# mirage/decompress

Hardware: AMD Instinct MI355X
Metric: MiB/s inflate over N zlib streams (uncompressed bytes / wall second) (higher is better)
Workload: dtype u8; 1 GPU; C2: 4096 x 256 KiB zlib streams per GPU, dynamic Huffman (libz level 6; even streams = slices of the reference's test/corpus, odd = order-2 Markov ASCII text, 64 symbols, seed 0xC2 + i, SURVEY 8(d)), Zl.Inf.Ns semantics, one stream per pair of wavefronts (decoder + copier); streams_per_gpu=4096, stream_bytes=262144, unique_streams=4096

## Files before the change

decompress_amd/csrc/inflate_util.hpp:

```cpp
#pragma once
#include <hip/hip_runtime.h>
#include <type_traits>
#include <stdint.h>

#include "mdeflate.h"

namespace md {
namespace wv {

constexpr int kWave = 64;
__device__ __forceinline__ uint32_t uni(uint32_t v) { return __builtin_amdgcn_readfirstlane(v); }

#define MD_LDS __attribute__((address_space(3)))
typedef MD_LDS uint32_t lds_u32;
typedef MD_LDS uint16_t lds_u16;
typedef MD_LDS uint8_t lds_u8;
typedef uint64_t u64_u __attribute__((aligned(1), may_alias));
typedef uint32_t u32_u __attribute__((aligned(1), may_alias));
typedef uint16_t u16_u __attribute__((aligned(1), may_alias));

enum { P_ENSURE = 0, P_DECODE1, P_DECODE2, P_EMIT_A, P_FAR, P_NEAR, P_ADLER, P_HEADER, P_NEAR_FAST, P_NEAR_SLOW, P_NEAR_UPD, P_NEAR_LOAD, P_HDR_LENS, P_HDR_LIT, P_FAR_REC, P_FAR_LOAD, P_WAIT_DEC, P_WAIT_COPY, P_COUNT };
enum { C_ROUNDS = 0, C_PASSES, C_LANES, C_TOKENS, C_SLOTS, C_NEAR_IT,
       C_END_CHAIN, C_END_FIT, C_END_RECORDS, C_END_STAGE, C_END_EOB, C_LONG_NEAR, C_FAR_SPILL, C_COUNT };
template <bool ON>
struct Prof {
  static constexpr bool on = true;
  uint64_t t0;
  uint64_t acc[P_COUNT];
  uint32_t cnt[C_COUNT];
  __device__ __forceinline__ void init() {
    for (int i = 0; i < P_COUNT; i++) acc[i] = 0;
    for (int i = 0; i < C_COUNT; i++) cnt[i] = 0;
    t0 = clock64();
  }
  __device__ __forceinline__ void tick(int i) {
    uint64_t t = clock64();
    acc[i] += t - t0;
    t0 = t;
  }
  __device__ __forceinline__ void tick_lds(int i) {
    __builtin_amdgcn_s_waitcnt(0xc07f);
    tick(i);
  }
  __device__ __forceinline__ void tick_all(int i) {
    __builtin_amdgcn_s_waitcnt(0);
    tick(i);
  }
  __device__ __forceinline__ void count(int i, uint32_t n = 1) { cnt[i] += n; }
};
template <>
struct Prof<false> {
  static constexpr bool on = false;
  __device__ __forceinline__ void init() {}
  __device__ __forceinline__ void tick(int) {}
  __device__ __forceinline__ void tick_lds(int) {}
  __device__ __forceinline__ void tick_all(int) {}
  __device__ __forceinline__ void count(int, uint32_t = 1) {}
};

__device__ __forceinline__ uint32_t wave_incl_scan(uint32_t x) {
  uint32_t v = x;
  v += (uint32_t)__builtin_amdgcn_update_dpp(0, (int)v, 0x111, 0xf, 0xf, false);
  v += (uint32_t)__builtin_amdgcn_update_dpp(0, (int)v, 0x112, 0xf, 0xf, false);
  v += (uint32_t)__builtin_amdgcn_update_dpp(0, (int)v, 0x114, 0xf, 0xf, false);
  v += (uint32_t)__builtin_amdgcn_update_dpp(0, (int)v, 0x118, 0xf, 0xf, false);
  v += (uint32_t)__builtin_amdgcn_update_dpp(0, (int)v, 0x142, 0xa, 0xf, false);
  v += (uint32_t)__builtin_amdgcn_update_dpp(0, (int)v, 0x143, 0xc, 0xf, false);
  return v;
}
__device__ __forceinline__ uint32_t wave_sum(uint32_t v) {
  return (uint32_t)__builtin_amdgcn_readlane((int)wave_incl_scan(v), 63);
}
__device__ __forceinline__ uint32_t wave_excl_scan(uint32_t v, uint32_t) { return wave_incl_scan(v) - v; }
__device__ __forceinline__ uint32_t wave_shr1(uint32_t v) { return (uint32_t)__builtin_amdgcn_update_dpp(0, (int)v, 0x138, 0xf, 0xf, false); }
__device__ __forceinline__ uint32_t rdlane(uint32_t v, uint32_t l) {
  return __builtin_amdgcn_readlane(v, __builtin_amdgcn_readfirstlane(l));
}

__device__ __forceinline__ uint64_t out_ld64(const uint8_t *p) {
  return __builtin_nontemporal_load(reinterpret_cast<const u64_u *>(p));
}
__device__ __forceinline__ uint32_t out_ld8(const uint8_t *p) { return __builtin_nontemporal_load(p); }
__device__ __forceinline__ uint64_t out_ld_guard(const uint8_t *g, uint32_t x, uint32_t n, uint32_t cap) {
  if (x + 8 <= cap) return out_ld64(g + x);
  uint64_t v = 0;
  for (uint32_t j = 0; j < n && j < 8; j++) v |= (uint64_t)out_ld8(g + x + j) << (8 * j);
  return v;
}
__device__ __forceinline__ uint64_t lds_ld64(const lds_u8 *p) { return *reinterpret_cast<const MD_LDS u64_u *>(p); }

__device__ __forceinline__ void lds_put(lds_u8 *p, uint64_t v, uint32_t n) {
  const uint32_t lo = (uint32_t)v, hi = (uint32_t)(v >> 32);
  if (n >= 4) {
    const uint32_t k = n - 4;
    const uint32_t t = k >= 4 ? hi : __builtin_amdgcn_alignbyte(hi, lo, k);
    *reinterpret_cast<MD_LDS u32_u *>(p) = lo;
    *reinterpret_cast<MD_LDS u32_u *>(p + k) = t;
  } else {
    *p = (uint8_t)lo;
    if (n > 1) *reinterpret_cast<MD_LDS u16_u *>(p + n - 2) = (uint16_t)(lo >> (8 * (n - 2)));
  }
}

}
}
```

decompress_amd/csrc/inflate_wave_core.hpp:

```cpp
#pragma once
#include <stdlib.h>
#include "inflate_util.hpp"
#include "internal.hpp"

#if !defined(MD_RMAX) || !defined(MD_STAGE)
#error "define MD_RMAX and MD_STAGE before inflate_wave_core.hpp"
#endif

namespace md {
namespace wv {

constexpr uint32_t S = 264;
constexpr uint32_t SMIN = 48;
constexpr uint32_t KMAX = 64;
#ifndef MD_EMIT_SPLIT
#define MD_EMIT_SPLIT 1
#endif
#if defined(MD_DEBUG_KNOWN_BOUNDS)
#undef MD_EMIT_SPLIT
#define MD_EMIT_SPLIT 0
#endif
#ifndef MD_SPLIT_B
#define MD_SPLIT_B 4
#endif
#ifndef MD_RUNIN_NUM
#define MD_RUNIN_NUM 3
#define MD_RUNIN_DEN 2
#endif
constexpr uint32_t RUNIN_NUM = MD_RUNIN_NUM, RUNIN_DEN = MD_RUNIN_DEN;
constexpr uint32_t PASSES = 5;
constexpr uint32_t PASS_BITS = 1600, PASSES_MAX = 16;
constexpr uint32_t RMAX = MD_RMAX;
constexpr uint32_t STAGE = MD_STAGE;
constexpr uint32_t WIN_WORDS = 544;

constexpr uint32_t kLitSize = 852, kDistSize = 592;
constexpr uint32_t kLitRootMax = 512;
constexpr uint32_t kLitSubB = 0;
constexpr uint32_t kDistB = kLitSize - kLitRootMax;
constexpr uint32_t kLitB = kDistB + kDistSize;
constexpr uint32_t kStopEobI = kLitB + kLitRootMax;
constexpr uint32_t kStopBadI = kStopEobI + 2;
constexpr uint32_t kLutWords = kStopBadI + 2;
constexpr uint32_t kTbMask = 0xffe00000u;
constexpr uint32_t kLoopy = 0x100u;
static_assert(kDistB % 2 == 0 && kLitB % 2 == 0 && kStopEobI % 2 == 0 && kLutWords == 1448, "even table bases");
constexpr uint32_t kStEob = 100, kStTrunc = 101;
constexpr uint32_t kCountMatch = 1u << 20;
constexpr uint32_t kNearBit = 0x8000u;

struct Mail {
  uint32_t emitted;
  uint32_t copied;
  uint32_t kind;
  uint32_t total;
  uint32_t x;
  uint32_t stuck;
  uint32_t a, b;
};
constexpr uint32_t kJobRound = 0, kJobStored = 1, kJobQuit = 2, kJobEmit = 3;
constexpr uint32_t kHxUni = 4 * 64;
struct Smem {
  uint32_t win[WIN_WORDS];
  uint32_t lut[kLutWords];
  uint32_t mrec[RMAX];
  uint16_t mpos[RMAX];
  alignas(16) uint8_t stage[STAGE + 16];
  uint16_t list[RMAX];
  Mail mail;
};
struct HScratch {
  uint8_t lens[384];
  uint16_t work[320];
  uint32_t ctr;
};
#if MD_RMAX == 576 && MD_STAGE == 5248
static_assert(sizeof(Smem) <= 17920, "9 streams (18 wavefronts) per CU: 160 KiB / 9, in whole 512-byte units");
#endif
static_assert(RMAX % 64 == 0 && STAGE % 16 == 0 && RMAX * 2 >= (kHxUni + 6) * 4, "record rows, staging chunks, the emit job's words in `list`");
constexpr uint32_t kHScratchAt = 1136;
static_assert(kHScratchAt >= 4 + 572 + 8 && kHScratchAt % 16 == 0 && kHScratchAt + sizeof(HScratch) <= WIN_WORDS * 4, "header scratch lives behind the header's bits");
typedef MD_LDS Smem lds_smem;
typedef MD_LDS HScratch lds_hscratch;
__device__ __forceinline__ lds_hscratch *hscratch_of(lds_smem *sm) {
  return reinterpret_cast<lds_hscratch *>(reinterpret_cast<lds_u8 *>(sm->win) + kHScratchAt);
}

__device__ __forceinline__ uint32_t mk_entry(uint32_t n, uint32_t xb, uint32_t val8, uint32_t nbits, uint32_t tb) {
  return n | (xb << 5) | (val8 << 9) | (nbits << 17) | (tb << 21);
}
__device__ __forceinline__ uint32_t e_n(uint32_t e) { return e & 31; }
__device__ __forceinline__ uint32_t e_xb(uint32_t e) { return (e >> 5) & 15; }
__device__ __forceinline__ uint32_t e_val(uint32_t e) { return (e >> 9) & 255; }
__device__ __forceinline__ uint32_t e_tb(uint32_t e) { return e >> 21; }
__device__ __forceinline__ bool e_link(uint32_t e) { return e_tb(e) < kLitB && e_tb(e) != kDistB; }
__device__ __forceinline__ uint32_t e_root(uint32_t lroot) { return mk_entry(0, 0, 0, lroot, kLitB); }
__device__ __forceinline__ uint32_t lit_leaf(uint32_t sym, uint32_t codelen, uint32_t lroot, uint32_t droot) {
  if (sym < 256) return mk_entry(codelen, 0, sym, lroot, kLitB);
  if (sym == 256) return mk_entry(codelen, 0, 0, 0, kStopEobI);
  const uint32_t l = (sym - 257) & 31;
  const uint32_t xb = (l >= 8 && l < 28) ? (l - 4) >> 2 : 0;
  const uint32_t base3 = l < 8 ? l : l < 28 ? (4 + (l & 3)) << xb : l == 28 ? 255 : 0;
  return mk_entry(codelen + xb, xb, base3, droot, kDistB);
}
__device__ __forceinline__ uint32_t dist_leaf(uint32_t dv, uint32_t codelen, uint32_t lroot) {
  dv &= 31;
  if (dv >= 30) return mk_entry(codelen, 0, 0, 0, kStopBadI);
  const uint32_t xb = dv >= 4 ? (dv - 2) >> 1 : 0;
  const uint32_t m = dv < 4 ? dv : ((dv & 1) | 2);
  return mk_entry(codelen + xb, xb, m, lroot, kLitB);
}
__device__ __forceinline__ uint32_t dist_value(uint32_t m, uint32_t xb, uint32_t x) { return (m << xb) + 1 + x; }

struct Window {
  uint32_t w[8], wx;
  uint32_t base;
#ifdef MD_DEBUG_KNOWN_BOUNDS
  uint32_t kb_round, kb_sid;
#endif
  __device__ __forceinline__ void fetch(const uint8_t *__restrict__ body, uint32_t nbytes, uint32_t b, uint32_t lane) {
    base = b;
    const uint32_t off = b + lane * 32;
#pragma unroll
    for (int k = 0; k < 8; k++) w[k] = 0;
    if (off + 32 <= nbytes) __builtin_memcpy(w, body + off, 32);
    else if (off < nbytes)
      for (uint32_t k = 0; k < 32 && off + k < nbytes; k++) w[k >> 2] |= (uint32_t)body[off + k] << (8 * (k & 3));
    wx = 0;
    if (lane < WIN_WORDS - 512) {
      const uint32_t ox = b + 2048 + lane * 4;
      if (ox + 4 <= nbytes) __builtin_memcpy(&wx, body + ox, 4);
      else if (ox < nbytes)
        for (uint32_t k = 0; k < 4 && ox + k < nbytes; k++) wx |= (uint32_t)body[ox + k] << (8 * k);
    }
  }
  __device__ __forceinline__ void put(lds_u32 *win, uint32_t lane) const {
    lds_u32 *dst = win + lane * 8;
#pragma unroll
    for (int k = 0; k < 8; k++) dst[k] = w[k];
    if (lane < WIN_WORDS - 512) win[512 + lane] = wx;
  }
  __device__ __forceinline__ void ensure(lds_u32 *win, const uint8_t *__restrict__ body, uint32_t nbytes, uint32_t b, uint32_t lane) {
    if (base != b) fetch(body, nbytes, b, lane);
    put(win, lane);
    base = 0xffffffffu;
  }
};
__device__ __forceinline__ uint32_t peek(const lds_u32 *win, uint32_t p) {
  const lds_u32 *q = reinterpret_cast<const lds_u32 *>(reinterpret_cast<const lds_u8 *>(win) + ((p >> 3) & ~3u));
  return __builtin_amdgcn_alignbit(q[1], q[0], p & 31);
}
__device__ __forceinline__ uint32_t lut_at(const lds_u32 *lut, uint32_t tb, uint32_t idx) {
  return *reinterpret_cast<const lds_u32 *>(reinterpret_cast<const lds_u8 *>(lut) + ((tb + idx) << 2));
}

struct UBits {
  const lds_u32 *win;
  uint64_t buf;
  uint32_t n;
  uint32_t wp;
  __device__ __forceinline__ void init(const lds_u32 *w, uint32_t bp) {
    win = w;
    wp = bp >> 5;
    buf = ((uint64_t)uni(win[wp]) | ((uint64_t)uni(win[wp + 1]) << 32)) >> (bp & 31);
    n = 64 - (bp & 31);
    wp += 2;
  }
  __device__ __forceinline__ uint32_t pos() const { return wp * 32 - n; }
  __device__ __forceinline__ void fill() {
    if (n <= 32) {
      buf |= (uint64_t)uni(win[wp]) << n;
      n += 32;
      wp++;
    }
  }
  __device__ __forceinline__ uint32_t peekb(uint32_t k) const { return (uint32_t)buf & ((1u << k) - 1); }
  __device__ __forceinline__ void drop(uint32_t k) {
    buf >>= k;
    n -= k;
  }
};

struct Canon {
  uint32_t cnt[16];
  uint32_t first[16];
  uint32_t offs[16];
  uint32_t max, min, root, left;
};
__device__ __forceinline__ uint32_t lane_rank(uint64_t m) {
  return __builtin_amdgcn_mbcnt_hi((uint32_t)(m >> 32), __builtin_amdgcn_mbcnt_lo((uint32_t)m, 0));
}
template <int K>
__device__ __forceinline__ void canon_counts(const uint32_t (&len)[K], uint32_t rootpref, Canon &c) {
#pragma unroll
  for (int l = 1; l < 16; l++) {
    uint32_t n = 0;
#pragma unroll
    for (int k = 0; k < K; k++) n += (uint32_t)__builtin_popcountll(__ballot(len[k] == (uint32_t)l));
    c.cnt[l] = n;
  }
  c.cnt[0] = 0;
  c.max = 0;
  c.min = 16;
#pragma unroll
  for (int l = 15; l >= 1; l--) {
    if (c.cnt[l] && c.max == 0) c.max = l;
    if (c.cnt[l]) c.min = l;
  }
  int left = 1;
  bool over = false;
  uint32_t code = 0, off = 0;
  c.first[0] = 0;
  c.offs[0] = 0;
#pragma unroll
  for (int l = 1; l < 16; l++) {
    left = (left << 1) - (int)c.cnt[l];
    over = over || left < 0;
    code = (code + c.cnt[l - 1]) << 1;
    c.first[l] = code;
    c.offs[l] = off;
    off += c.cnt[l];
  }
  c.left = over ? 0xffffffffu : (uint32_t)left;
  uint32_t root = rootpref;
  if (root > c.max) root = c.max;
  if (root < c.min) root = c.min;
  c.root = root;
}

template <int K, class LEAF>
__device__ __forceinline__ bool build_walk(const uint32_t (&len)[K], const Canon &c, lds_u32 *lut, uint32_t tb0, uint32_t sub0,
                                           uint32_t size, lds_hscratch *hs, uint32_t lane, uint32_t zero_entry, LEAF leaf) {
  const uint32_t root = c.root, rmask = (1u << root) - 1;
  uint32_t rev[K];
#pragma unroll
  for (int k = 0; k < K; k++) rev[k] = 0;
#pragma unroll
  for (int l = 1; l < 16; l++) {
    if (c.cnt[l]) {
      uint32_t base = 0;
#pragma unroll
      for (int k = 0; k < K; k++) {
        const uint64_t m = __ballot(len[k] == (uint32_t)l);
        if (len[k] == (uint32_t)l) {
          const uint32_t rank = base + lane_rank(m);
          rev[k] = __brev(c.first[l] + rank) >> (32 - l);
          hs->work[c.offs[l] + rank] = (uint16_t)(lane + 64 * k);
        }
        base += (uint32_t)__builtin_popcountll(m);
      }
    }
  }
  const uint32_t nroot = 1u << root;
  for (uint32_t i = lane; i < nroot; i += kWave) lut[tb0 + i] = 0;
  if (lane == 0) hs->ctr = 0;
  if (c.max > root) {
#pragma unroll
    for (int k = 0; k < K; k++)
      if (len[k] > root)
        __hip_atomic_fetch_max(&lut[tb0 + (rev[k] & rmask)], len[k], __ATOMIC_RELAXED, __HIP_MEMORY_SCOPE_WORKGROUP);
  }
  for (uint32_t i = lane; i < nroot; i += kWave) {
    const uint32_t v = lut[tb0 + i];
    uint32_t e;
    if (v) {
      const uint32_t sub = v - root;
      const uint32_t off = __hip_atomic_fetch_add(&hs->ctr, 1u << sub, __ATOMIC_RELAXED, __HIP_MEMORY_SCOPE_WORKGROUP);
      e = mk_entry(root, 0, 0, sub, (sub0 + off) & 2047);
    } else {
      const uint32_t cw = __brev(i) >> (32 - root);
      uint32_t fl = 0, ft = 0;
#pragma unroll
      for (int l = 15; l >= 1; l--) {
        if (c.cnt[l] && (uint32_t)l <= root) {
          const uint32_t t = (cw >> (root - l)) - c.first[l];
          if (t < c.cnt[l]) {
            fl = l;
            ft = c.offs[l] + t;
          }
        }
      }
      e = fl ? leaf((uint32_t)hs->work[ft], fl) : zero_entry;
    }
    lut[tb0 + i] = e;
  }
  const uint32_t used = nroot + uni(hs->ctr);
  if (used > size) return false;
  if (c.max > root) {
#pragma unroll
    for (int k = 0; k < K; k++) {
      if (len[k] > root) {
        const uint32_t link = lut[tb0 + (rev[k] & rmask)];
        const uint32_t sub = (link >> 17) & 15, tb = link >> 21;
        const uint32_t e = leaf(lane + 64 * k, len[k] - root);
        for (uint32_t j = rev[k] >> root; j < (1u << sub); j += 1u << (len[k] - root)) lut[tb + j] = e;
      }
    }
  }
  return true;
}

constexpr uint64_t kZig0 = 16ull | 17ull << 5 | 18ull << 10 | 0ull << 15 | 8ull << 20 | 7ull << 25 | 9ull << 30 | 6ull << 35 |
                           10ull << 40 | 5ull << 45 | 11ull << 50 | 4ull << 55;
constexpr uint64_t kZig1 = 12ull | 3ull << 5 | 13ull << 10 | 2ull << 15 | 14ull << 20 | 1ull << 25 | 15ull << 30;

template <class PF>
__device__ __noinline__ int dynamic_tables(lds_smem *sm, uint32_t bp_arg, uint32_t tot_arg, uint32_t lane, uint32_t *bp_out,
                                           uint32_t *lroot_out, PF &pf) {
  const uint32_t bp = uni(bp_arg), tot = uni(tot_arg);
  const lds_u32 *win = (const lds_u32 *)sm->win;
  lds_hscratch *hs = hscratch_of(sm);
  UBits ub;
  ub.init(win, bp);
  if ((int32_t)(tot - ub.pos()) < 14) return MD_UNEXPECTED_END_OF_INPUT;
  const uint32_t hlit = ub.peekb(5) + 257;
  ub.drop(5);
  const uint32_t hdist = ub.peekb(5) + 1;
  ub.drop(5);
  const uint32_t hclen = ub.peekb(4) + 4;
  ub.drop(4);
  uint32_t cl[1] = {0};
  for (uint32_t i = 0; i < hclen; i++) {
    ub.fill();
    if ((int32_t)(tot - ub.pos()) < 3) return MD_UNEXPECTED_END_OF_INPUT;
    const uint32_t v = ub.peekb(3);
    ub.drop(3);
    const uint32_t z = (uint32_t)((i < 12 ? kZig0 >> (5 * i) : kZig1 >> (5 * (i - 12))) & 31);
    if (lane == z) cl[0] = v;
  }
  Canon cc;
  canon_counts<1>(cl, 7, cc);
  uint32_t cmaxl, t_lo, t_hi;
  if (cc.max == 0) {
    cmaxl = 1;
    t_lo = lane == 0 ? (1u << 8) : 0xffffu;
    t_hi = 0xffffu;
  } else {
    if (cc.left != 0) return MD_INVALID_DICTIONARY;
    cmaxl = cc.max;
#pragma unroll
    for (int l = 1; l < 8; l++) {
      const uint64_t m = __ballot(cl[0] == (uint32_t)l);
      if (cl[0] == (uint32_t)l) hs->work[cc.offs[l] + lane_rank(m)] = (uint16_t)lane;
    }
    uint32_t t[2];
#pragma unroll
    for (int h = 0; h < 2; h++) {
      const uint32_t i = lane + 64 * h;
      const uint32_t cw = __brev(i & ((1u << cmaxl) - 1)) >> (32 - cmaxl);
      uint32_t fl = 0, ft = 0;
#pragma unroll
      for (int l = 7; l >= 1; l--) {
        if (cc.cnt[l] && (uint32_t)l <= cmaxl) {
          const uint32_t x = (cw >> (cmaxl - l)) - cc.first[l];
          if (x < cc.cnt[l]) {
            fl = l;
            ft = cc.offs[l] + x;
          }
        }
      }
      t[h] = fl ? ((uint32_t)hs->work[ft] | (fl << 8)) : 0xffffu;
    }
    t_lo = t[0];
    t_hi = t[1];
  }
  const uint32_t max_res = hlit + hdist;
  for (uint32_t x = lane; x < 384; x += kWave) hs->lens[x] = 0;
  auto run_lengths = [&](auto checked) -> int {
    constexpr bool CHECK = decltype(checked)::value;
    uint32_t i = 0, prev = 0;
    while (i < max_res) {
      ub.fill();
      if (CHECK && (int32_t)(tot - ub.pos()) < (int32_t)cmaxl) return MD_UNEXPECTED_END_OF_INPUT;
      const uint32_t idx = ub.peekb(cmaxl);
      const uint32_t e_lo = __builtin_amdgcn_readlane(t_lo, idx & 63), e_hi = __builtin_amdgcn_readlane(t_hi, idx & 63);
      const uint32_t e = idx < 64 ? e_lo : e_hi;
      if (e == 0xffffu) return MD_INVALID_DICTIONARY;
      const uint32_t sym = e & 0xff;
      ub.drop(e >> 8);
      if (sym < 16) {
        hs->lens[i] = (uint8_t)sym;
        prev = sym;
        i++;
      } else {
        const uint32_t nb = sym == 16 ? 2 : sym == 17 ? 3 : 7;
        if (sym == 16 && i == 0) return MD_INVALID_DICTIONARY;
        ub.fill();
        if (CHECK && (int32_t)(tot - ub.pos()) < (int32_t)nb) return MD_UNEXPECTED_END_OF_INPUT;
        const uint32_t copy = ub.peekb(nb) + (sym == 18 ? 11 : 3);
        ub.drop(nb);
        const uint32_t val = sym == 16 ? prev : 0;
        if (i + copy > max_res) return MD_INVALID_DICTIONARY;
        if (val)
          for (uint32_t x = lane; x < copy; x += kWave) hs->lens[i + x] = (uint8_t)val;
        prev = val;
        i += copy;
      }
    }
    return MD_OK;
  };
  {
    const bool plenty = (int32_t)(tot - ub.pos()) >= 316 * 14 + 64;
    const int rc = plenty ? run_lengths(std::false_type{}) : run_lengths(std::true_type{});
    if (rc != MD_OK) return rc;
  }
  *bp_out = ub.pos();
  pf.tick_lds(P_HDR_LENS);
  if (uni(hs->lens[256]) == 0) return MD_INVALID_DICTIONARY;
  uint32_t ll[5], dl[1];
#pragma unroll
  for (int k = 0; k < 5; k++) ll[k] = lane + 64 * k < hlit ? (uint32_t)hs->lens[lane + 64 * k] : 0u;
  dl[0] = lane < hdist ? (uint32_t)hs->lens[hlit + lane] : 0u;
  Canon cl_, cd_;
  canon_counts<5>(ll, 9, cl_);
  canon_counts<1>(dl, 6, cd_);
  if (cl_.left == 0xffffffffu || (cl_.left > 0 && cl_.max != 1)) return MD_INVALID_DICTIONARY;
  const uint32_t lroot = cl_.root;
  uint32_t droot;
  lds_u32 *lut = (lds_u32 *)sm->lut;
  if (cd_.max == 0) {
    droot = 1;
  } else {
    if (cd_.left == 0xffffffffu || (cd_.left > 0 && cd_.max != 1)) return MD_INVALID_DICTIONARY;
    droot = cd_.root;
  }
  if (!build_walk<5>(ll, cl_, lut, kLitB, kLitSubB, kLitSize, hs, lane, e_root(lroot),
                     [=](uint32_t sym, uint32_t codelen) { return lit_leaf(sym, codelen, lroot, droot); }))
    return MD_INVALID_DICTIONARY;
  pf.tick_lds(P_HDR_LIT);
  if (cd_.max == 0) {
    if (lane == 0) {
      lut[kDistB] = dist_leaf(0, 1, lroot);
      lut[kDistB + 1] = mk_entry(0, 0, 0, 0, kStopBadI);
    }
  } else if (!build_walk<1>(dl, cd_, lut, kDistB, kDistB + (1u << droot), kDistSize, hs, lane, e_root(lroot),
                            [=](uint32_t sym, uint32_t codelen) { return dist_leaf(sym, codelen, lroot); }))
    return MD_INVALID_DICTIONARY;
  const bool loopy = cl_.left > 0 || (cd_.max != 0 && cd_.left > 0);
  *lroot_out = lroot | (loopy ? kLoopy : 0u);
  return MD_OK;
}

__device__ __noinline__ void fixed_tables(lds_smem *sm, uint32_t lane, uint32_t *lroot_out) {
  lds_hscratch *hs = hscratch_of(sm);
  uint32_t ll[5], dl[1];
#pragma unroll
  for (int k = 0; k < 5; k++) {
    const uint32_t n = lane + 64 * k;
    ll[k] = n < 144 ? 8 : n < 256 ? 9 : n < 280 ? 7 : n < 288 ? 8 : 0;
  }
  dl[0] = lane < 32 ? 5 : 0;
  Canon cl_, cd_;
  canon_counts<5>(ll, 9, cl_);
  canon_counts<1>(dl, 6, cd_);
  const uint32_t lroot = cl_.root, droot = cd_.root;
  lds_u32 *lut = (lds_u32 *)sm->lut;
  build_walk<5>(ll, cl_, lut, kLitB, kLitSubB, kLitSize, hs, lane, e_root(lroot),
                [=](uint32_t sym, uint32_t codelen) { return lit_leaf(sym, codelen, lroot, droot); });
  build_walk<1>(dl, cd_, lut, kDistB, kDistB + (1u << droot), kDistSize, hs, lane, e_root(lroot),
                [=](uint32_t sym, uint32_t codelen) { return dist_leaf(sym, codelen, lroot); });
  *lroot_out = lroot;
}

struct Cursor {
  uint32_t w0, w1, w2, wa;
  __device__ __forceinline__ void init(const lds_u32 *win, uint32_t p) {
    wa = (p >> 5) << 2;
    const lds_u32 *q = reinterpret_cast<const lds_u32 *>(reinterpret_cast<const lds_u8 *>(win) + wa);
    w0 = q[0];
    w1 = q[1];
    w2 = q[2];
  }
  __device__ __forceinline__ uint32_t peek(uint32_t p) const { return __builtin_amdgcn_alignbit(w1, w0, p); }
  __device__ __forceinline__ void seek(const lds_u32 *win, uint32_t pn) {
    const uint32_t wan = (pn >> 5) << 2;
    const bool ge = wan != wa;
    w0 = ge ? w1 : w0;
    w1 = ge ? w2 : w1;
    wa = wan;
    w2 = *reinterpret_cast<const lds_u32 *>(reinterpret_cast<const lds_u8 *>(win) + wa + 8);
  }
};
__device__ __forceinline__ uint32_t lut_step(const lds_u32 *lut, uint32_t e, uint32_t w) {
  return lut_at(lut, e >> 21, __builtin_amdgcn_ubfe(w, 0, e >> 17));
}

template <bool COUNT, bool BUDGET, bool MID = false>
__device__ __forceinline__ void sync_pass(const lds_u32 *win, const lds_u32 *lut, uint32_t lroot, bool go, uint32_t start,
                                          uint32_t limit, uint32_t &end, uint32_t &stop, uint32_t &nb, uint32_t mthr = 0,
                                          uint32_t *midp = nullptr, uint32_t *midcnt = nullptr) {
  if (go) {
    uint32_t p = start, e = e_root(lroot), cnt = 0;
    uint32_t mp = 0xffffffffu, mc = 0;
    bool got = false;
    if (MID && start >= mthr) {
      mp = start;
      got = true;
    }
    if (p < limit) {
      const uint32_t thr = (kLitB << 21) | limit;
      uint32_t slot = 0, key;
      Cursor c;
      c.init(win, start);
      do {
        const uint32_t w = c.peek(p);
        const uint32_t en = lut_step(lut, e, w);
        const uint32_t n = e_n(en);
        if (COUNT) {
          const uint32_t xb = e_xb(en);
          const uint32_t len1 = e_val(en) + __builtin_amdgcn_ubfe(w, n - xb, xb) + (kCountMatch + 2);
          cnt += (e_tb(en) == kLitB ? 1u : 0u) + (e_tb(en) == kDistB ? len1 : 0u);
        }
        p += n;
        if (MID) {
          const bool cross = (e_tb(en) == kLitB) & !got & (p >= mthr);
          mp = cross ? p : mp;
          mc = cross ? cnt : mc;
          got = got | cross;
        }
        c.seek(win, p);
        e = en;
        key = (en & kTbMask) | p;
        if (BUDGET && ++slot >= KMAX && e_tb(en) == kLitB) break;
      } while (key < thr);
    }
    end = p;
    stop = e_tb(e) >= kStopEobI ? e_tb(e) : 0u;
    if (COUNT) nb = cnt;
    if (MID) {
      *midp = mp;
      *midcnt = mc;
    }
  }
}

struct LaneOut {
  uint32_t endp;
  uint32_t stopc;
  uint32_t bytes;
  uint32_t nm;
};

__device__ __noinline__ uint32_t slow_token(const lds_u32 *win, const lds_u32 *lut, uint32_t lroot, uint32_t ptok, uint32_t q,
                                            uint32_t tot, uint32_t cap) {
  uint32_t p = ptok;
  uint32_t w = peek(win, p);
  uint32_t e = lut_step(lut, e_root(lroot), w);
  if (e_link(e)) {
    p += e_n(e);
    w = peek(win, p);
    e = lut_step(lut, e, w);
  }
  uint32_t n = e_n(e), xb = e_xb(e), ntb = e_tb(e);
  uint32_t pn = p + n;
  if (pn > tot) return MD_UNEXPECTED_END_OF_INPUT;
  if (ntb == kStopEobI) return kStEob | (pn << 8);
  if (ntb != kDistB) {
    if (q >= cap) return MD_UNEXPECTED_END_OF_OUTPUT;
    return kStTrunc;
  }
  const uint32_t mlen = e_val(e) + 3 + __builtin_amdgcn_ubfe(w, n - xb, xb);
  p = pn;
  w = peek(win, p);
  e = lut_step(lut, e, w);
  if (e_tb(e) == kStopBadI && e_n(e) == 0) return MD_INVALID_DISTANCE_CODE;
  if (e_link(e)) {
    p += e_n(e);
    w = peek(win, p);
    e = lut_step(lut, e, w);
  }
  n = e_n(e), xb = e_xb(e);
  pn = p + n;
  if (pn > tot) return MD_UNEXPECTED_END_OF_INPUT;
  if (e_tb(e) == kStopBadI) return MD_INVALID_DISTANCE_CODE;
  const uint32_t d = dist_value(e_val(e), xb, __builtin_amdgcn_ubfe(w, n - xb, xb));
  const uint32_t lim = q < 32768u ? q : 32768u;
  if (d > lim) return MD_INVALID_DISTANCE;
  if (mlen > cap - q) return MD_UNEXPECTED_END_OF_OUTPUT;
  return kStTrunc;
}

template <bool CHECKED, bool BUDGET>
__device__ __forceinline__ void emit_pass(const lds_u32 *win, const lds_u32 *lut, uint32_t lroot, lds_u32 *mrec,
                                          lds_u16 *mpos, lds_u8 *stage, uint32_t rec0, uint32_t tot, bool go, uint32_t start,
                                          uint32_t limit, uint32_t q0, uint32_t rb, uint32_t R0, uint32_t cap, LaneOut &lo) {
  uint32_t p = start, ptok = start, e = e_root(lroot);
  uint32_t q = q0, rec = rec0, mlen = 0;
  bool stopped = false;
  const uint32_t qlim = rb + STAGE - 16;
  const uint32_t qmax = cap < qlim ? cap : qlim;
  if (go && p < limit) {
    const uint32_t thr = (kLitB << 21) | limit;
    uint32_t slot = 0, key;
    Cursor c;
    c.init(win, start);
    do {
      const uint32_t w = c.peek(p);
      const uint32_t en = lut_step(lut, e, w);
      const uint32_t n = e_n(en), xb = e_xb(en), ntb = e_tb(en);
      const uint32_t x = __builtin_amdgcn_ubfe(w, n - xb, xb);
      const uint32_t pn = p + n;
      const bool to_root = ntb == kLitB, is_len = ntb == kDistB;
      const bool mat = to_root & (mlen != 0), lit = to_root & (mlen == 0);
      const uint32_t d1 = (e_val(en) << xb) + x;
      if (CHECKED) {
        const uint32_t lim = q < 32768u ? q : 32768u;
        const uint32_t need = mat ? mlen : 1u;
        stopped = (ntb >= kStopEobI) | (pn > tot) | (mat & (d1 >= lim)) | (to_root & (q + need > qmax));
        if (stopped) break;
      }
      stage[lit ? q - rb : STAGE + 15] = (uint8_t)(en >> 9);
      if (mat) {
        mrec[rec] = ((mlen - 3) << 16) | ((q - d1 + mlen > R0 + 1) ? kNearBit : 0u) | d1;
        mpos[rec] = (uint16_t)(q - rb);
        rec++;
      }
      q += to_root ? (mlen > 1u ? mlen : 1u) : 0u;
      mlen = is_len ? e_val(en) + 3 + x : to_root ? 0u : mlen;
      p = pn;
      ptok = to_root ? pn : ptok;
      c.seek(win, p);
      e = en;
      key = (en & kTbMask) | p;
      if (BUDGET && ++slot >= KMAX && to_root) break;
    } while (key < thr);
    if (!CHECKED) stopped = e_tb(e) >= kStopEobI;
  }
  uint32_t stopc = 0, endp = p;
  if (go && stopped) {
    const uint32_t r = slow_token(win, lut, lroot, ptok, q, tot, cap);
    stopc = r & 0xffu;
    endp = stopc == kStEob ? r >> 8 : ptok;
  }
  if (go) {
    lo.endp = endp;
    lo.stopc = stopc;
    lo.bytes = q - q0;
    lo.nm = rec - rec0;
  }
}

}
}
```

Baseline: 249,200 MiB/s.

## Decode dynamic Huffman header from registers instead of LDS

The dynamic-header bit reader now loads up to 128 window words into two VGPRs per lane and reads them back with readlane, replacing scalar LDS loads on every fill. Code-length-code fields are decoded in parallel, with each lane picking its own 3-bit field through an inverse zigzag table. Run-length decoded code lengths are written into registers with writelane and lane masks rather than into an LDS byte array, and the distance lengths are realigned with ds_bpermute. This removes LDS round-trips and waits from the serial header decode, at the cost of more register pressure and some readlane/writelane overhead.

```diff
diff --git a/decompress_amd/csrc/inflate_util.hpp b/decompress_amd/csrc/inflate_util.hpp
--- a/decompress_amd/csrc/inflate_util.hpp
+++ b/decompress_amd/csrc/inflate_util.hpp
@@ -77,6 +77,9 @@
   return __builtin_amdgcn_readlane(v, __builtin_amdgcn_readfirstlane(l));
 }
 
+extern "C" __device__ uint32_t md_llvm_writelane(uint32_t v, uint32_t l, uint32_t old) __asm("llvm.amdgcn.writelane.i32");
+__device__ __forceinline__ uint32_t wrlane(uint32_t old, uint32_t v, uint32_t l) { return md_llvm_writelane(v, l, old); }
+
 __device__ __forceinline__ uint64_t out_ld64(const uint8_t *p) {
   return __builtin_nontemporal_load(reinterpret_cast<const u64_u *>(p));
 }
diff --git a/decompress_amd/csrc/inflate_wave_core.hpp b/decompress_amd/csrc/inflate_wave_core.hpp
--- a/decompress_amd/csrc/inflate_wave_core.hpp
+++ b/decompress_amd/csrc/inflate_wave_core.hpp
@@ -70,7 +70,6 @@
   Mail mail;
 };
 struct HScratch {
-  uint8_t lens[384];
   uint16_t work[320];
   uint32_t ctr;
 };
@@ -78,8 +77,16 @@
 static_assert(sizeof(Smem) <= 17920, "9 streams (18 wavefronts) per CU: 160 KiB / 9, in whole 512-byte units");
 #endif
 static_assert(RMAX % 64 == 0 && STAGE % 16 == 0 && RMAX * 2 >= (kHxUni + 6) * 4, "record rows, staging chunks, the emit job's words in `list`");
+constexpr uint32_t kHdrBitsMax = 14 + 19 * 3 + 316 * 7;
+constexpr uint32_t kHdrReuseBits = 4096;
+constexpr uint32_t kHdrWordMax = (kHdrReuseBits + 3) / 32;
+constexpr uint32_t kHdrWords = 128;
+static_assert(31 + kHdrBitsMax + 14 + 64 <= kHdrWords * 32, "start phase, header, a last peek and the bit buffer's read-ahead");
 constexpr uint32_t kHScratchAt = 1136;
-static_assert(kHScratchAt >= 4 + 572 + 8 && kHScratchAt % 16 == 0 && kHScratchAt + sizeof(HScratch) <= WIN_WORDS * 4, "header scratch lives behind the header's bits");
+static_assert(kHScratchAt >= (kHdrWordMax + 1) * 4 + (kHdrBitsMax + 7) / 8 + 8 && kHScratchAt % 16 == 0 &&
+                  kHScratchAt + sizeof(HScratch) <= WIN_WORDS * 4,
+              "header scratch lives behind the header's bits");
+static_assert(kHdrWordMax + kHdrWords <= WIN_WORDS, "the header's register copy stays inside the window");
 typedef MD_LDS Smem lds_smem;
 typedef MD_LDS HScratch lds_hscratch;
 __device__ __forceinline__ lds_hscratch *hscratch_of(lds_smem *sm) {
@@ -155,21 +162,35 @@
 }
 
 struct UBits {
-  const lds_u32 *win;
+  uint32_t hw[2];
+  uint32_t w0;
   uint64_t buf;
   uint32_t n;
   uint32_t wp;
-  __device__ __forceinline__ void init(const lds_u32 *w, uint32_t bp) {
-    win = w;
-    wp = bp >> 5;
-    buf = ((uint64_t)uni(win[wp]) | ((uint64_t)uni(win[wp + 1]) << 32)) >> (bp & 31);
-    n = 64 - (bp & 31);
+  __device__ __forceinline__ uint32_t word(uint32_t i) const {
+    const uint32_t a = __builtin_amdgcn_readlane(hw[0], i & 63), b = __builtin_amdgcn_readlane(hw[1], i & 63);
+    return i < 64 ? a : b;
+  }
+  __device__ __forceinline__ void load(const lds_u32 *win, uint32_t bp, uint32_t lane) {
+    w0 = bp >> 5;
+#pragma unroll
+    for (int j = 0; j < 2; j++) {
+      const uint32_t w = w0 + lane + 64 * j;
+      hw[j] = win[w < WIN_WORDS ? w : WIN_WORDS - 1];
+    }
+    seek(bp & 31);
+  }
+  __device__ __forceinline__ void seek(uint32_t p) {
+    wp = p >> 5;
+    buf = ((uint64_t)word(wp) | ((uint64_t)word(wp + 1) << 32)) >> (p & 31);
+    n = 64 - (p & 31);
     wp += 2;
   }
-  __device__ __forceinline__ uint32_t pos() const { return wp * 32 - n; }
+  __device__ __forceinline__ uint32_t hpos() const { return wp * 32 - n; }
+  __device__ __forceinline__ uint32_t pos() const { return w0 * 32 + hpos(); }
   __device__ __forceinline__ void fill() {
     if (n <= 32) {
-      buf |= (uint64_t)uni(win[wp]) << n;
+      buf |= (uint64_t)word(wp) << n;
       n += 32;
       wp++;
     }
@@ -229,8 +250,14 @@
 }
 
 template <int K, class LEAF>
-__device__ __forceinline__ bool build_walk(const uint32_t (&len)[K], const Canon &c, lds_u32 *lut, uint32_t tb0, uint32_t sub0,
+__device__ __forceinline__ bool build_walk(const uint32_t (&len_in)[K], const Canon &c, lds_u32 *lut, uint32_t tb0, uint32_t sub0,
                                            uint32_t size, lds_hscratch *hs, uint32_t lane, uint32_t zero_entry, LEAF leaf) {
+  uint32_t len[K];
+#pragma unroll
+  for (int k = 0; k < K; k++) {
+    len[k] = len_in[k];
+    asm volatile("" : "+v"(len[k]));
+  }
   const uint32_t root = c.root, rmask = (1u << root) - 1;
   uint32_t rev[K];
 #pragma unroll
@@ -303,6 +330,15 @@
 constexpr uint64_t kZig0 = 16ull | 17ull << 5 | 18ull << 10 | 0ull << 15 | 8ull << 20 | 7ull << 25 | 9ull << 30 | 6ull << 35 |
                            10ull << 40 | 5ull << 45 | 11ull << 50 | 4ull << 55;
 constexpr uint64_t kZig1 = 12ull | 3ull << 5 | 13ull << 10 | 2ull << 15 | 14ull << 20 | 1ull << 25 | 15ull << 30;
+constexpr uint32_t zig_at(uint32_t i) { return (uint32_t)((i < 12 ? kZig0 >> (5 * i) : kZig1 >> (5 * (i - 12))) & 31); }
+constexpr uint64_t zig_inverse(uint32_t z0, uint32_t z1) {
+  uint64_t r = 0;
+  for (uint32_t z = z0; z < z1; z++)
+    for (uint32_t i = 0; i < 19; i++)
+      if (zig_at(i) == z) r |= (uint64_t)i << (5 * (z - z0));
+  return r;
+}
+constexpr uint64_t kZigInv0 = zig_inverse(0, 12), kZigInv1 = zig_inverse(12, 19);
 
 template <class PF>
 __device__ __noinline__ int dynamic_tables(lds_smem *sm, uint32_t bp_arg, uint32_t tot_arg, uint32_t lane, uint32_t *bp_out,
@@ -311,7 +347,7 @@
   const lds_u32 *win = (const lds_u32 *)sm->win;
   lds_hscratch *hs = hscratch_of(sm);
   UBits ub;
-  ub.init(win, bp);
+  ub.load(win, bp, lane);
   if ((int32_t)(tot - ub.pos()) < 14) return MD_UNEXPECTED_END_OF_INPUT;
   const uint32_t hlit = ub.peekb(5) + 257;
   ub.drop(5);
@@ -319,14 +355,17 @@
   ub.drop(5);
   const uint32_t hclen = ub.peekb(4) + 4;
   ub.drop(4);
-  uint32_t cl[1] = {0};
-  for (uint32_t i = 0; i < hclen; i++) {
-    ub.fill();
-    if ((int32_t)(tot - ub.pos()) < 3) return MD_UNEXPECTED_END_OF_INPUT;
-    const uint32_t v = ub.peekb(3);
-    ub.drop(3);
-    const uint32_t z = (uint32_t)((i < 12 ? kZig0 >> (5 * i) : kZig1 >> (5 * (i - 12))) & 31);
-    if (lane == z) cl[0] = v;
+  if ((int32_t)(tot - ub.pos()) < (int32_t)(3 * hclen)) return MD_UNEXPECTED_END_OF_INPUT;
+  uint32_t cl[1];
+  {
+    const uint32_t fp = ub.hpos(), w = fp >> 5, sh = fp & 31;
+    const uint32_t f0 = __builtin_amdgcn_readlane(ub.hw[0], w), f1 = __builtin_amdgcn_readlane(ub.hw[0], w + 1),
+                   f2 = __builtin_amdgcn_readlane(ub.hw[0], w + 2);
+    const uint64_t fields = ((((uint64_t)f1 << 32) | f0) >> sh) | (((uint64_t)f2 << 1) << (63 - sh));
+    const uint32_t z = lane < 19 ? lane : 18;
+    const uint32_t i = (uint32_t)((z < 12 ? kZigInv0 >> (5 * z) : kZigInv1 >> (5 * (z - 12))) & 31);
+    cl[0] = (lane < 19 && i < hclen) ? (uint32_t)(fields >> (3 * i)) & 7u : 0u;
+    ub.seek(fp + 3 * hclen);
   }
   Canon cc;
   canon_counts<1>(cl, 7, cc);
@@ -365,7 +404,14 @@
     t_hi = t[1];
   }
   const uint32_t max_res = hlit + hdist;
-  for (uint32_t x = lane; x < 384; x += kWave) hs->lens[x] = 0;
+  uint32_t lr[5] = {0, 0, 0, 0, 0};
+  uint32_t cur = 0, kc = 0;
+  auto next_reg = [&]() {
+#pragma unroll
+    for (int k = 0; k < 5; k++) lr[k] = kc == (uint32_t)k ? cur : lr[k];
+    cur = 0;
+    kc++;
+  };
   auto run_lengths = [&](auto checked) -> int {
     constexpr bool CHECK = decltype(checked)::value;
     uint32_t i = 0, prev = 0;
@@ -378,8 +424,9 @@
       if (e == 0xffffu) return MD_INVALID_DICTIONARY;
       const uint32_t sym = e & 0xff;
       ub.drop(e >> 8);
+      uint32_t val = 0;
       if (sym < 16) {
-        hs->lens[i] = (uint8_t)sym;
+        cur = wrlane(cur, sym, i & 63);
         prev = sym;
         i++;
       } else {
@@ -389,12 +436,15 @@
         if (CHECK && (int32_t)(tot - ub.pos()) < (int32_t)nb) return MD_UNEXPECTED_END_OF_INPUT;
         const uint32_t copy = ub.peekb(nb) + (sym == 18 ? 11 : 3);
         ub.drop(nb);
-        const uint32_t val = sym == 16 ? prev : 0;
+        val = sym == 16 ? prev : 0;
         if (i + copy > max_res) return MD_INVALID_DICTIONARY;
-        if (val)
-          for (uint32_t x = lane; x < copy; x += kWave) hs->lens[i + x] = (uint8_t)val;
+        if (val) cur = lane - (i & 63) < copy ? val : cur;
         prev = val;
         i += copy;
+      }
+      while ((i >> 6) != kc) {
+        next_reg();
+        if (val) cur = lane < i - 64 * kc ? val : 0u;
       }
     }
     return MD_OK;
@@ -405,12 +455,16 @@
     if (rc != MD_OK) return rc;
   }
   *bp_out = ub.pos();
+  next_reg();
   pf.tick_lds(P_HDR_LENS);
-  if (uni(hs->lens[256]) == 0) return MD_INVALID_DICTIONARY;
+  if (__builtin_amdgcn_readlane(lr[4], 0) == 0) return MD_INVALID_DICTIONARY;
   uint32_t ll[5], dl[1];
 #pragma unroll
-  for (int k = 0; k < 5; k++) ll[k] = lane + 64 * k < hlit ? (uint32_t)hs->lens[lane + 64 * k] : 0u;
-  dl[0] = lane < hdist ? (uint32_t)hs->lens[hlit + lane] : 0u;
+  for (int k = 0; k < 5; k++) ll[k] = lane + 64 * k < hlit ? lr[k] : 0u;
+  {
+    const uint32_t up = (uint32_t)__builtin_amdgcn_ds_bpermute((int)(((lane + hlit - 256) & 63) << 2), (int)lr[4]);
+    dl[0] = lane < hdist ? up : 0u;
+  }
   Canon cl_, cd_;
   canon_counts<5>(ll, 9, cl_);
   canon_counts<1>(dl, 6, cd_);
```

Result: no change. 248,400 MiB/s (-0.3%).
